# s-elkazdadi/ddp-pinocchio

Measured on AMD Instinct MI355X. Metric: DDP iterations/sec (fwd+bwd sweep), Talos nq=38 T=200, higher is better.
Workload: dtype f64

## Files before the change

ddp_pinocchio_amd/csrc/ctx.hip:

```cpp
#include <math.h>
#include <stdio.h>
#include <stdlib.h>
#include <string.h>

#include <limits>
#include <new>

#include "internal.h"

extern "C" int ddp_hip_abi_version(void) { return DDP_HIP_ABI_VERSION; }

extern "C" const char* ddp_hip_strerror(int code) {
  switch (code) {
    case DDP_HIP_OK: return "ok";
    case DDP_HIP_EV_LLT_RESTART: return "backward sweep restarted after a non-positive LLT pivot";
    case DDP_HIP_EV_LINESEARCH_FLOOR: return "line search reached step < 1e-10";
    case DDP_HIP_E_ARG: return "invalid argument";
    case DDP_HIP_E_HIP: return "HIP runtime error";
    case DDP_HIP_E_NODEVICE: return "no HIP device (there is no CPU fallback)";
    case DDP_HIP_E_UNSUPPORTED: return "unsupported configuration";
    case DDP_HIP_E_MAX_RESTARTS: return "backward sweep exceeded max_restarts";
    case DDP_HIP_E_COMM: return "RCCL error";
    default: return "unknown";
  }
// ... 157 lines not shown
         s == DDP_HIP_SEQ_FB_VAL || s == DDP_HIP_SEQ_FB_JAC || s == DDP_HIP_SEQ_X || s == DDP_HIP_SEQ_U ||
         s == DDP_HIP_SEQ_X_NEW || s == DDP_HIP_SEQ_U_NEW || is_trace_seq(s);
}

__global__ void fill_kernel(double* p, int64_t n, double v) {
  int64_t i = (int64_t)blockIdx.x * blockDim.x + threadIdx.x;
  int64_t stride = (int64_t)gridDim.x * blockDim.x;
  for (; i < n; i += stride) p[i] = v;
}

static int fill_device(ddp_hip_ctx* ctx, double* p, int64_t n, double v) {
  if (n <= 0) return DDP_HIP_OK;
  if (v == 0.0) {
    HIP_TRY(hipMemsetAsync(p, 0, (size_t)n * sizeof(double), ctx->stream));
    return DDP_HIP_OK;
  }
  int64_t blocks = (n + 255) / 256;
  if (blocks > 2048) blocks = 2048;
  hipLaunchKernelGGL(fill_kernel, dim3((unsigned)blocks), dim3(256), 0, ctx->stream, p, n, v);
  HIP_TRY(hipGetLastError());
  return DDP_HIP_OK;
}

static DevSwitches read_switches() {
  auto on = [](const char* name) { return getenv(name) != nullptr; };
  auto knob = [](const char* name, int lo, int hi) { const char* ev = getenv(name); const int v = ev ? atoi(ev) : 0; return v >= lo && v <= hi ? v : 0; };
  DevSwitches sw;
  sw.generic_bwd = on("DDP_HIP_GENERIC_BWD");
  sw.k3_no_sym = on("DDP_HIP_K3_NO_SYM");
  sw.k3_no_half = on("DDP_HIP_K3_NO_HALF");
  sw.k3_no_pack = on("DDP_HIP_K3_NO_PACK");
  sw.fxx_full = on("DDP_HIP_FXX_FULL");
  sw.no_static = on("DDP_HIP_NO_STATIC");
  sw.no_qcache = on("DDP_HIP_NO_QCACHE");
  sw.cfg_full_aba = on("DDP_HIP_CFG_FULL_ABA");
  sw.ana_own_aba = on("DDP_HIP_ANA_OWN_ABA");
  sw.ana_split = on("DDP_HIP_ANA_SPLIT");
  sw.ana_eq_kernel = on("DDP_HIP_ANA_EQ_KERNEL");
  sw.bwd_no_graph = on("DDP_HIP_BWD_NO_GRAPH");
  sw.solve_sync = on("DDP_HIP_SOLVE_SYNC");
  sw.fwd_no_pipe = on("DDP_HIP_FWD_NO_PIPE");
  sw.bwd_cbx = knob("DDP_HIP_BWD_CBX", 1, 8);
  sw.bwd_cbu = knob("DDP_HIP_BWD_CBU", 1, 16);
  sw.qws_bt = knob("DDP_HIP_QWS_BT", 16, 65536);
  sw.ana_bt = knob("DDP_HIP_ANA_BT", 1, 65536);
  return sw;
}

static int cost_block_setup(ddp_hip_ctx* ctx, int term, int32_t items) {
  CostBlock& k = ctx->cost[term];
  const int64_t slots = ctx->d.batch * (ctx->d.T + 1) * k.max_items;
  for (int s = 0; s < k.desc->nside; ++s) {
    const int64_t words = slots * k.desc->unit[s];
    const int fill = k.desc->fill[s];
    if (!k.side[s]) HIP_TRY(hipMalloc(&k.side[s], sizeof(double) * (size_t)words));
    if (fill == FILL_QUAT) {
      std::vector<double> qt((size_t)words, 0.0);
      for (size_t i = 3; i < qt.size(); i += 4) qt[i] = 1.0;
      HIP_TRY(hipMemcpyAsync(k.side[s], qt.data(), sizeof(double) * qt.size(), hipMemcpyHostToDevice, ctx->stream));
      HIP_TRY(hipStreamSynchronize(ctx->stream));
    } else {
      const int rc = fill_device(ctx, k.side[s], words, fill == FILL_NEG_INF ? -INFINITY : fill == FILL_POS_INF ? INFINITY : 0.0);
      if (rc != DDP_HIP_OK) return rc;
    }
  }
  k.items = items;
  k.live = false;
  return DDP_HIP_OK;
}

extern "C" int ddp_hip_create(const ddp_hip_problem* prob, int device, uint32_t flags, ddp_hip_ctx** out) {
// ... 566 lines not shown
```

ddp_pinocchio_amd/csrc/internal.h:

```cpp
#pragma once

#include <hip/hip_runtime.h>
#include <stdint.h>

#include <vector>

#include "cost_block.h"
#include "ddp_hip/ddp_hip.h"

#define DDP_MAXJ DDP_HIP_MAX_JOINTS

struct DevModel {
  int32_t kind, nv;
  int32_t ff, nj, nq, pad0_;
  double mass, length;
  double gravity[3];
  double dt, c;
  int32_t parent[DDP_MAXJ];
  int32_t jtype[DDP_MAXJ];
  double axis[DDP_MAXJ][3];
  double Rp[DDP_MAXJ][9];
  double pp[DDP_MAXJ][3];
  double I6[DDP_MAXJ][21];
  int32_t has_child[DDP_MAXJ];
// ... 23 lines not shown
};

struct BwdJob {
  int32_t kind;
  int32_t c0, cn;
  int32_t pad_;
};

struct DevSwitches {
  bool generic_bwd = false;
  bool k3_no_sym = false;
  bool k3_no_half = false;
  bool k3_no_pack = false;
  bool fxx_full = false;
  bool no_static = false;
  bool no_qcache = false;
  bool cfg_full_aba = false;
  bool ana_own_aba = false;
  bool ana_split = false;
  bool ana_eq_kernel = false;
  bool bwd_no_graph = false;
  bool solve_sync = false;
  bool fwd_no_pipe = false;
  int32_t bwd_cbx = 0, bwd_cbu = 0;
  int64_t qws_bt = 0;
  int64_t ana_bt = 0;
};

struct SweepPlan {
  bool fast;
  bool sym_ok;
  bool sym;
  int32_t half_mode;
  bool packed;
};

enum class LinFirst : int32_t {
  Base,
  AnalyticSmall,
  AnalyticWave,
  AnalyticFF,
  FdStatic,
  FdGeneric,
};
enum class LinSecond : int32_t {
  None,
  Zeros,
  Mode2Static,
  Mode2Caches,
  Mode2Plain,
  Mode1Small,
  Mode1Wave,
};
enum class LinEq : int32_t {
  None,
  PerLane,
  Analytic,
  Chain,
};
enum class LinEqJac : int32_t { None, Fd, FfLookahead };
enum class LinEqSecond : int32_t { None, Zeros, Mode2, Mode1Small, Mode1Wave };
struct LinPlan {
  int32_t refuse = 0;
  int32_t nj = 0;
  int32_t topo = 0;
  LinFirst first = LinFirst::Base;
  LinSecond second = LinSecond::None;
  LinEq eq = LinEq::None;
  LinEqJac eq_jac = LinEqJac::None;
  LinEqSecond eq_second = LinEqSecond::None;
  bool eq_inline = false;
  bool accel_static = false;
  bool accel_with_u = false;
  bool m1_fused = false;
  int32_t ncfg = 0, nvcfg = 0;
  bool has_tensors = false;
  bool skip_top = false;
  bool skip_qv_mirror = false;
  bool pack = false;
  bool ws_lin = false, ws_qws = false, ws_qws2 = false;
  bool ws_ana_T = false, ws_ana_M = false, ws_ana_M0 = false, ws_ana_A = false, ws_ana_F = false;
  bool ws_eq = false;
  bool ana_sliced = false;
  int64_t eq_fxk_off = 0, eq_c_off = 0, eq_words = 0;
  int32_t lin_path = 0, first_order = 0;
};
LinPlan lin_plan_decide(const DevModel& m, const Dims& d, uint32_t flags, const DevSwitches& sw, int topo_id, bool sweep_sym_ok);

enum class TensorOrigin : int32_t {
  Unknown,
  Symmetric,
  Stencil,
  Analytic1,
};
struct TensorState {
  TensorOrigin origin = TensorOrigin::Unknown;
  bool mirror_pending = false;
  bool packed = false;
};

struct LinCall {
  bool ana_A_fresh = false;
  bool ana_M0_fresh = false;
  bool fuu_zero = false;
};

struct ProfSlot {
  std::vector<hipEvent_t> starts, stops;
  size_t used = 0;
// ... 32 lines not shown
  struct BwdGraph { const void* key_x = nullptr; uint64_t key_misc = 0; hipGraphExec_t exec = nullptr; hipGraph_t graph = nullptr; };
  BwdGraph bwd_graph[4];
  int bwd_graph_next = 0;

  double* fw_x = nullptr;
  double* fw_u = nullptr;
  double* fw_dcost = nullptr;
  double* fw_cost = nullptr;
  double* fw_cost_old = nullptr;
  double* step_d = nullptr;
  int32_t* fw_state_d = nullptr;
  double* fw_dcost_acc_d = nullptr;
  int32_t n_alpha_max = 8;
  double* pick_pair_d = nullptr;

  double* eq_ws = nullptr;
  double* lin_ws = nullptr;
  LinPlan plan;
  double* lin_qws = nullptr;
  int64_t lin_qws_bt = 0;
  double* lin_qws2 = nullptr;
  hipStream_t lin_stream2 = nullptr;
  hipEvent_t lin_ev_up[2] = {nullptr, nullptr}, lin_ev_dn[2] = {nullptr, nullptr};
  double* ana_T = nullptr;
  double* ana_M = nullptr;
  double* ana_F = nullptr;
  double* ana_M0 = nullptr;
  double* ana_A = nullptr;
  int64_t ana_nbt = 0;

  std::vector<int32_t> active_h;
  bool all_active = true;

  CostBlock cost[COST_COUNT];
  int32_t fc_nf = 0;
  int32_t fc_joint[DDP_HIP_MAX_COST_FRAMES] = {};
  double fc_off[DDP_HIP_MAX_COST_FRAMES][3] = {};
  int32_t ob_np = 0, ob_no = 0;
  int32_t ob_joint[DDP_HIP_MAX_COLLISION_POINTS] = {};
  double ob_off[DDP_HIP_MAX_COLLISION_POINTS][3] = {};
  double ob_radius[DDP_HIP_MAX_COLLISION_POINTS] = {};
  int32_t ob_kind[DDP_HIP_MAX_OBSTACLES] = {};
  double* ob_clear_d = nullptr;

  bool box_dirty = false;

  bool async_mode = false;
  uint32_t profile_mask = 0;
  ProfSlot prof[DDP_HIP_K_COUNT];
};

#define HIP_TRY(expr)                                   \
  do {                                                  \
    hipError_t e__ = (expr);                            \
    if (e__ != hipSuccess) { (void)hipGetLastError(); return DDP_HIP_E_HIP; } \
  } while (0)

#define END_SYNC(ctx) do { if (!(ctx)->async_mode) HIP_TRY(hipStreamSynchronize((ctx)->stream)); } while (0)

void prof_begin(ddp_hip_ctx* ctx, int kid, hipStream_t stream = nullptr);
void prof_end(ddp_hip_ctx* ctx, int kid, hipStream_t stream = nullptr);

int bwd_setup(ddp_hip_ctx* ctx);
SweepPlan sweep_plan(const ddp_hip_ctx* ctx);
void bwd_teardown(ddp_hip_ctx* ctx);
int bwd_lds_check(const ddp_hip_ctx* ctx);
int box_check(ddp_hip_ctx* ctx);
int fwd_setup(ddp_hip_ctx* ctx);
bool fwd_lat_supported(const ddp_hip_ctx* ctx);
void fwd_teardown(ddp_hip_ctx* ctx);
int lin_setup(ddp_hip_ctx* ctx);
int tensors_written_outside(ddp_hip_ctx* ctx, int seq);
int lin_materialize_fxx(ddp_hip_ctx* ctx);
void lin_teardown(ddp_hip_ctx* ctx);

int pick_local_launch(ddp_hip_ctx* ctx, int64_t rank, int64_t nranks, double* out_pair, hipStream_t stream);
int pick_final_launch(const double* pairs, int G, double* out_pair, hipStream_t stream);

static inline int64_t seq_block_offset_regular(int64_t t, int64_t stride) { return t * stride; }
```

ddp_pinocchio_amd/csrc/lin.hip:

```cpp
#include <float.h>
#include <math.h>
#include <stdlib.h>

#include "com_cost.h"
#include "frame_cost.h"
#include "frame_vel_cost.h"
#include "internal.h"
#include "lin_common.h"
#include "obstacle_cost.h"
#include "rbd.h"
#include "rbd_deriv.h"
#include "state_limits.h"

namespace {



__global__ void lin_cost_kernel(LinParams p) {
  const int64_t T = p.d.T;
  const int64_t bt = blockIdx.x;
  const int b = (int)(bt / T);
  const int64_t t = bt % T;
  const int n = (int)p.d.n, m = (int)p.d.m;
  const double c = p.model->c;
// ... 1138 lines not shown
        const int rc_ = lin_analytic_launch(ctx, p, call, 0, LIN_ANA_F | (m1_next ? LIN_ANA_ACCEL : 0) | (m1_next && eq_stage ? LIN_ANA_EQ << 4 : 0));
        if (rc_ != DDP_HIP_OK) return rc_;
        break;
      }
      case LinFirst::FdStatic: {
        build_caches();
        const int rc_ = lin_static_launch(ctx, p, StaticLevel::FirstOrder);
        if (rc_ != DDP_HIP_OK) return rc_;
        break;
      }
      case LinFirst::FdGeneric:
        hipLaunchKernelGGL((lin_first_kernel<NJ>), dim3(blocks_for(BT * W)), dim3(LBS), 0, ctx->stream, p);
        break;
    }
    prof_end(ctx, DDP_HIP_K_LIN_FIRST);
  }
  if (second_stage) {
    const int64_t P = (int64_t)W * (W - 1) / 2, TRI = (int64_t)nv * (nv - 1) / 2, Pv = (int64_t)nv * nv + TRI, Pu = 2 * (int64_t)nv * nv + TRI;
    prof_begin(ctx, DDP_HIP_K_LIN_SECOND);
    switch (pl.second) {
      case LinSecond::None: break;
      case LinSecond::Mode2Static:
        build_caches();
        for (StaticLevel level : {StaticLevel::UDiagonal, StaticLevel::Torque, StaticLevel::Velocity, StaticLevel::Configuration}) {
          const int rc_ = lin_static_launch(ctx, p, level);
          if (rc_ != DDP_HIP_OK) return rc_;
        }
        break;
      case LinSecond::Mode2Caches:
        build_caches();
        hipLaunchKernelGGL((lin_diag_kernel<NJ>), dim3(blocks_for(BT * W)), dim3(LBS), 0, ctx->stream, p);
        hipLaunchKernelGGL((lin_offdiag_kernel<NJ, 3>), dim3(blocks_for(BT * Pu)), dim3(LBS), 0, ctx->stream, p);
        hipLaunchKernelGGL((lin_offdiag_kernel<NJ, 2>), dim3(blocks_for(BT * Pv)), dim3(LBS), 0, ctx->stream, p);
        hipLaunchKernelGGL((lin_offdiag_kernel<NJ, 1>), dim3(blocks_for(BT * TRI)), dim3(LBS), 0, ctx->stream, p);
        break;
      case LinSecond::Mode2Plain:
        hipLaunchKernelGGL((lin_diag_kernel<NJ>), dim3(blocks_for(BT * W)), dim3(LBS), 0, ctx->stream, p);
        hipLaunchKernelGGL((lin_offdiag_kernel<NJ, 0>), dim3(blocks_for(BT * P)), dim3(LBS), 0, ctx->stream, p);
        break;
      case LinSecond::Mode1Small:
        if constexpr (small) hipLaunchKernelGGL((second_m1_kernel<NJ>), dim3(blocks_for(BT * W)), dim3(LBS), 0, ctx->stream, p, 0);
        break;
      case LinSecond::Mode1Wave:
        if (!m1_fused) { const int rc_ = lin_analytic_launch(ctx, p, call, 1, LIN_ANA_F); if (rc_ != DDP_HIP_OK) return rc_; }
        break;
      case LinSecond::Zeros:
        HIP_TRY(hipMemsetAsync(p.fxx, 0, sizeof(double) * (size_t)(ctx->seq[DDP_HIP_SEQ_FXX].size * d.batch), ctx->stream));
        HIP_TRY(hipMemsetAsync(p.fux, 0, sizeof(double) * (size_t)(ctx->seq[DDP_HIP_SEQ_FUX].size * d.batch), ctx->stream));
        HIP_TRY(hipMemsetAsync(p.fuu, 0, sizeof(double) * (size_t)(ctx->seq[DDP_HIP_SEQ_FUU].size * d.batch), ctx->stream));
        break;
    }
    prof_end(ctx, DDP_HIP_K_LIN_SECOND);
  }
  if (eq_stage) {
    switch (pl.eq) {
      case LinEq::None: break;
      case LinEq::PerLane:
        if constexpr (small) hipLaunchKernelGGL((eq_first_kernel<NJ>), dim3(blocks_for(BT)), dim3(LBS), 0, ctx->stream, p);
        break;
      case LinEq::Analytic: {
        const int rc_ = lin_analytic_launch(ctx, p, call, 0, LIN_ANA_EQ);
        if (rc_ != DDP_HIP_OK) return rc_;
        break;
      }
      case LinEq::Chain: {
        const int K = ctx->model_h.eq_advance;
        if (K < 1) return DDP_HIP_E_UNSUPPORTED;
        hipLaunchKernelGGL((eq_chain_kernel<NJ>), dim3(blocks_for(BT)), dim3(LBS), 0, ctx->stream, p);
        if (pl.eq_jac == LinEqJac::Fd) hipLaunchKernelGGL((eq_fdjac_kernel<NJ>), dim3(blocks_for(BT * (K - 1) * d.n)), dim3(LBS), 0, ctx->stream, p);
        else if (pl.eq_jac == LinEqJac::FfLookahead) { const int rc_ = lin_analytic_ff_lookahead(ctx, p); if (rc_ != DDP_HIP_OK) return rc_; }
        hipLaunchKernelGGL(eq_combine_kernel, dim3((unsigned)BT), dim3(256), sizeof(double) * (size_t)(2 * d.emax * d.n), ctx->stream, p);
        break;
      }
    }
// ... 20 lines not shown
  return DDP_HIP_OK;
}

void tensors_end_second(ddp_hip_ctx* ctx, const LinParams& p, const LinCall& call) {
  TensorState& t = ctx->tensors;
  if (ctx->model_h.fd_mode == 1) t.origin = call.fuu_zero ? TensorOrigin::Analytic1 : TensorOrigin::Unknown;
  else t.origin = p.skip_top ? TensorOrigin::Stencil : TensorOrigin::Symmetric;
  t.mirror_pending = p.skip_qv_mirror != 0;
  t.packed = p.pack != 0;
}

}

int lin_setup(ddp_hip_ctx* ctx) {
  const Dims& d = ctx->d;
  const int topo_id = ctx->model_h.kind == DDP_HIP_MODEL_TREE ? lin_static_supported(ctx->model_h) : 0;
  ctx->plan = lin_plan_decide(ctx->model_h, d, ctx->flags, ctx->sw, topo_id, sweep_plan(ctx).sym_ok);
  const LinPlan& pl = ctx->plan;
  if (pl.refuse) return pl.refuse;
  if (pl.ws_lin)
    HIP_TRY(hipMalloc(&ctx->lin_ws, sizeof(double) * (size_t)(d.batch * d.T * ((int64_t)pl.ncfg * d.nv * rbd::QC_STRIDE + (int64_t)pl.nvcfg * d.nv * rbd::VC_STRIDE))));
  if (pl.ws_qws) {
    const int64_t BT = d.batch * d.T;
    int64_t slice = 1024;
    if (ctx->sw.qws_bt) slice = ctx->sw.qws_bt;
    ctx->lin_qws_bt = BT < slice ? BT : slice;
    HIP_TRY(hipMalloc(&ctx->lin_qws, sizeof(double) * (size_t)(ctx->lin_qws_bt * lin_static_ws_per_bt(ctx->model_h))));
    if (pl.ws_qws2) {
      HIP_TRY(hipMalloc(&ctx->lin_qws2, sizeof(double) * (size_t)(ctx->lin_qws_bt * lin_static_ws_per_bt(ctx->model_h))));
      HIP_TRY(hipStreamCreateWithFlags(&ctx->lin_stream2, hipStreamNonBlocking));
      for (int k = 0; k < 2; ++k) {
        HIP_TRY(hipEventCreateWithFlags(&ctx->lin_ev_up[k], hipEventDisableTiming));
        HIP_TRY(hipEventCreateWithFlags(&ctx->lin_ev_dn[k], hipEventDisableTiming));
      }
    }
  }
  { const int rc_ = lin_analytic_setup(ctx); if (rc_ != DDP_HIP_OK) return rc_; }
  if (pl.ws_eq) HIP_TRY(hipMalloc(&ctx->eq_ws, sizeof(double) * (size_t)pl.eq_words));
  if (pl.eq == LinEq::Chain) {
    const size_t lds = sizeof(double) * (size_t)(2 * d.emax * d.n);
    if (lds > 64 * 1024) HIP_TRY(hipFuncSetAttribute(reinterpret_cast<const void*>(&eq_combine_kernel), hipFuncAttributeMaxDynamicSharedMemorySize, (int)lds));
  }
  return DDP_HIP_OK;
}
void lin_teardown(ddp_hip_ctx* ctx) {
  lin_analytic_teardown(ctx);
  for (int k = 0; k < 2; ++k) {
    if (ctx->lin_ev_up[k]) (void)hipEventDestroy(ctx->lin_ev_up[k]);
    if (ctx->lin_ev_dn[k]) (void)hipEventDestroy(ctx->lin_ev_dn[k]);
  }
  if (ctx->lin_stream2) (void)hipStreamDestroy(ctx->lin_stream2);
  if (ctx->lin_qws2) (void)hipFree(ctx->lin_qws2);
  if (ctx->lin_qws) (void)hipFree(ctx->lin_qws);
  if (ctx->eq_ws) (void)hipFree(ctx->eq_ws);
  if (ctx->lin_ws) (void)hipFree(ctx->lin_ws);
}

extern "C" int ddp_hip_linearize_stages(ddp_hip_ctx* ctx, uint32_t stages) {
  if (!ctx) return DDP_HIP_E_ARG;
  HIP_TRY(hipSetDevice(ctx->device));
  LinParams p = make_params(ctx);
  LinCall call;
  const bool second = (stages & DDP_HIP_LIN_SECOND) && p.has_tensors;
  if (second) { const int rc_ = tensors_begin_second(ctx, p, call); if (rc_ != DDP_HIP_OK) return rc_; }
  int rc;
  switch (ctx->plan.nj) {
    case 1: rc = run_linearize<1>(ctx, p, call, stages); break;
    case 6: rc = run_linearize<6>(ctx, p, call, stages); break;
    case 38: rc = run_linearize<38>(ctx, p, call, stages); break;
    default: rc = run_linearize<64>(ctx, p, call, stages); break;
  }
  if (rc != DDP_HIP_OK) return rc;
  END_SYNC(ctx);
  if (second) tensors_end_second(ctx, p, call);
  return DDP_HIP_OK;
}

int tensors_written_outside(ddp_hip_ctx* ctx, int seq) {
  if (seq != DDP_HIP_SEQ_FXX && seq != DDP_HIP_SEQ_FUX && seq != DDP_HIP_SEQ_FUU) return DDP_HIP_OK;
  TensorState& t = ctx->tensors;
  if (t.packed) { const int rc_ = lin_materialize_fxx(ctx); if (rc_ != DDP_HIP_OK) return rc_; }
  if (seq == DDP_HIP_SEQ_FUX) {
    t.origin = (t.origin == TensorOrigin::Symmetric || t.origin == TensorOrigin::Stencil) ? TensorOrigin::Symmetric : TensorOrigin::Unknown;
    return DDP_HIP_OK;
  }
// ... 35 lines not shown
```

ddp_pinocchio_amd/csrc/lin_common.h:

```cpp
#pragma once
#include "internal.h"

struct LinParams {
  Dims d;
  const DevModel* model;
  const int64_t* ne;
  const int64_t* Epre;
  const double* target;
  const double *x, *u;
  double *lfx, *lfxx, *lx, *lu, *lxx, *lux, *luu;
  double *f_val, *fx, *fu, *fxx, *fux, *fuu;
  double *eq_val, *eq_x, *eq_u, *eq_xx, *eq_ux, *eq_uu;
  int32_t has_tensors;
  double *eq_xk, *eq_fxk, *eq_c;
  double* vcache;
  double* qcache;
  int32_t skip_qv_mirror;
  int32_t skip_top;
  int32_t pack;
  double* accel_out;
  int32_t ncfg, nvcfg;
  const double *xref, *wx, *uref, *wu;
};

constexpr int LBS = 64;

int lin_static_supported(const DevModel& m);
enum class StaticLevel {
  Caches,
  FirstOrder,
  UDiagonal,
  Torque,
  Velocity,
  Configuration,
  AccelX,
  AccelXU,
};
int lin_static_launch(ddp_hip_ctx* ctx, const LinParams& p, StaticLevel level);
int64_t lin_static_ws_per_bt(const DevModel& m);

int lin_analytic_setup(ddp_hip_ctx* ctx);
void lin_analytic_teardown(ddp_hip_ctx* ctx);
constexpr int LIN_ANA_F = 1, LIN_ANA_EQ = 2;
constexpr int LIN_ANA_ACCEL = 4;
int lin_analytic_launch(ddp_hip_ctx* ctx, const LinParams& p, LinCall& call, int stage, int flags);
int lin_analytic_ff_lookahead(ddp_hip_ctx* ctx, const LinParams& p);
```

ddp_pinocchio_amd/csrc/lin_plan.cpp:

```cpp
#include "internal.h"

LinPlan lin_plan_decide(const DevModel& m, const Dims& d, uint32_t flags, const DevSwitches& sw, int topo_id, bool sweep_sym_ok) {
  LinPlan pl;
  const bool tree = m.kind == DDP_HIP_MODEL_TREE, ff = m.ff != 0, fo_fd = m.first_order_fd != 0;
  const bool tensors = !(flags & DDP_HIP_FLAG_NO_TENSORS);
  const bool analytic = tree && !fo_fd;
  const int mode = m.fd_mode;
  const int64_t nv = d.nv, K = m.eq_advance;
  pl.has_tensors = tensors;
  pl.nj = nv <= 1 ? 1 : (nv <= 6 && !ff) ? 6 : nv <= 38 ? 38 : 64;
  const bool small = pl.nj <= 6;
  const bool wave = analytic && !small && !ff;

  if (mode == 1 && fo_fd && tensors) pl.refuse = DDP_HIP_E_UNSUPPORTED;
  if (analytic && ff && nv > 38) pl.refuse = DDP_HIP_E_UNSUPPORTED;
  if (wave && m.max_level_width > 64) pl.refuse = DDP_HIP_E_UNSUPPORTED;
  if (wave && d.Etot > 0 && (K < 1 || K > 2)) pl.refuse = DDP_HIP_E_UNSUPPORTED;

  const int topo = (tree && !ff && !sw.no_static) ? topo_id : 0;
  const bool stencil_caches = tree && mode == 2 && tensors && !ff && !sw.no_qcache;
  const bool accel = topo && wave && mode == 1 && tensors && !sw.ana_own_aba;
  if (stencil_caches) { pl.ncfg = (int32_t)nv + 1; pl.nvcfg = 2 * (int32_t)nv + 1; }
  else if ((topo && fo_fd) || accel) { pl.ncfg = 1; pl.nvcfg = 1; }
  pl.ws_lin = pl.ncfg > 0;
// ... 17 lines not shown
  const bool m1_wave = wave && pl.second == LinSecond::Mode1Wave;
  pl.ana_sliced = analytic && !small;
  pl.ws_ana_T = wave && sw.ana_split;
  pl.ws_ana_M = wave && (sw.ana_split || (m1_wave && d.Etot > 0));
  pl.ws_ana_M0 = m1_wave && !sw.ana_split;
  pl.ws_ana_A = pl.accel_static = accel;
  pl.accel_with_u = accel && d.Etot > 0;
  pl.ws_ana_F = m1_wave && d.Etot > 0;

  pl.ws_eq = d.Etot > 0 && tree && (fo_fd || ff);
  if (d.Etot > 0) {
    pl.eq = (small && !pl.ws_eq) ? LinEq::PerLane : wave ? LinEq::Analytic : LinEq::Chain;
    if (pl.eq == LinEq::Chain && K > 1) pl.eq_jac = fo_fd ? LinEqJac::Fd : LinEqJac::FfLookahead;
    pl.eq_second = !tensors ? LinEqSecond::None : mode == 0 ? LinEqSecond::Zeros : mode == 2 ? LinEqSecond::Mode2
                   : small ? LinEqSecond::Mode1Small : LinEqSecond::Mode1Wave;
    pl.m1_fused = m1_wave;
    pl.eq_inline = m1_wave && !sw.ana_split && m.eq_kind == DDP_HIP_EQ_CONFIG && !sw.ana_eq_kernel;
  }
  if (pl.ws_eq) {
    pl.eq_fxk_off = d.batch * d.T * K * d.nx;
    pl.eq_c_off = pl.eq_fxk_off + d.batch * d.T * (K > 1 ? K - 1 : 0) * d.n * d.n;
    pl.eq_words = pl.eq_c_off + d.batch * d.T * d.emax * d.n;
  }
  pl.lin_path = tree ? 1 + pl.topo : 0;
  pl.first_order = tree ? (fo_fd ? 1 : 2) : 0;
  return pl;
}

#ifdef LIN_PLAN_TABLE
#include <stdio.h>

int main() {
  static const char* const sw_names[] = {"none", "generic_bwd", "k3_no_sym", "k3_no_half", "fxx_full", "no_static", "no_qcache",
                                         "cfg_full_aba", "ana_own_aba", "ana_split", "ana_eq_kernel", "bwd_no_graph", "solve_sync"};
  printf("kind nv ff fo_fd mode tensors etot eq_kind K matched sw sym_ok created refuse nj topo first second eq eq_jac eq_second "
         "eq_inline accel_static accel_with_u m1_fused ncfg nvcfg has_tensors skip_top skip_qv_mirror pack ws_lin ws_qws ws_qws2 ws_ana_T "
         "ws_ana_M ws_ana_M0 ws_ana_A ws_ana_F ws_eq ana_sliced eq_fxk_off eq_c_off eq_words lin_path first_order\n");
  printf("#");
  for (const char* s : sw_names) printf(" %s", s);
  printf("\n");
  const int nvs[] = {1, 6, 7, 38, 39, 64};
  for (int kind : {DDP_HIP_MODEL_PENDULUM, DDP_HIP_MODEL_TREE})
  for (int nv : nvs) for (int ff = 0; ff < 2; ++ff) for (int fo = 0; fo < 2; ++fo) for (int mode = 0; mode < 3; ++mode)
  for (int tensors = 0; tensors < 2; ++tensors) for (int etot = 0; etot < 2; ++etot)
  for (int eqk : {DDP_HIP_EQ_NONE, DDP_HIP_EQ_CONFIG, DDP_HIP_EQ_FRAME}) for (int K = 1; K <= 3; ++K)
  for (int matched = 0; matched < 2; ++matched) for (int s = 0; s < 13; ++s) {
    DevModel m{};
    m.kind = kind; m.nv = nv; m.ff = ff; m.nj = ff ? nv - 5 : nv; m.nq = nv + ff;
    m.first_order_fd = fo; m.fd_mode = mode; m.eq_kind = eqk; m.eq_advance = K; m.max_level_width = 4;
    Dims d{};
    d.T = 3; d.batch = 2; d.nv = nv; d.n = 2 * nv; d.m = nv; d.nx = 2 * nv + ff;
    d.emax = etot ? (eqk == DDP_HIP_EQ_CONFIG ? nv : 3) : 0; d.Etot = etot ? d.emax * d.T : 0;
    DevSwitches sw;
    bool* const sws[] = {nullptr, &sw.generic_bwd, &sw.k3_no_sym, &sw.k3_no_half, &sw.fxx_full, &sw.no_static, &sw.no_qcache,
                         &sw.cfg_full_aba, &sw.ana_own_aba, &sw.ana_split, &sw.ana_eq_kernel, &sw.bwd_no_graph, &sw.solve_sync};
// ... 16 lines not shown
```

ddp_pinocchio_amd/csrc/lin_static.hip:

```cpp
#include <float.h>
#include <math.h>
#include <stdlib.h>

#include <type_traits>
#include <utility>

#include "internal.h"
#include "lin_common.h"
#include "rbd.h"

#ifndef DEV_NO_EMIT
#define DEV_NO_EMIT 0
#endif
namespace {

struct TopoTalos38 {
  static constexpr int N = 38;
  static constexpr int parent[N] = {-1, 0, 1, 2, 3, 4,
                                    5, 6, 7, 8, 9, 10,
                                    5, 12, 13, 14, 15, 16,
                                    5, 18,
                                    19, 20, 21, 22, 23, 24, 25, 26,
                                    19, 28, 29, 30, 31, 32, 33, 34,
                                    19, 36};
// ... 667 lines not shown
  }
#pragma unroll
  for (int k = 0; k < 6; ++k) vel[k] += vJ[k];
  rbd::crm(vel, vJ, cb);
  double sum = 0;
#pragma unroll
  for (int k = 0; k < 6; ++k) { ap[k] += cb[k]; sum += U[k] * ap[k]; }
  double ui;
  if constexpr (C::UQS == 0) ui = s.uu[K]; else ui = c.uq[K * C::UQS];
  const double qd = (ui - sum) * dinv;
  if constexpr (C::UQS == 0) s.uu[K] = qd; else c.uq[K * C::UQS] = qd;
  if constexpr (has_child<T>(K)) {
#pragma unroll
    for (int k = 0; k < 6; ++k) { s.vel[K][k] = vel[k]; s.acc[K][k] = ap[k]; }
    s.acc[K][o] += a[0] * qd; s.acc[K][o + 1] += a[1] * qd; s.acc[K][o + 2] += a[2] * qd;
  }
  __builtin_amdgcn_sched_barrier(0);
}
template <class T, class C, int... Ks>
__device__ __forceinline__ void vel_down_all(const C& c, VelState<T>& s, std::integer_sequence<int, Ks...>) {
  (vel_down<T, Ks>(c, s), ...);
}

template <class T, bool ROWS>
__global__ __launch_bounds__(LBS, ROWS ? 3 : 2) void lin_static_vel_kernel(LinParams p) {
  constexpr int nv = T::N, n = 2 * nv;
  constexpr int TRI = nv * (nv - 1) / 2, GU = (TRI + LBS - 1) / LBS, G = ROWS ? nv : GU;
  const int64_t bt = blockIdx.x / G;
  const int g = (int)(blockIdx.x % G);
  const int lane = threadIdx.x;
  const int64_t Tn = p.d.T;
  const int b = (int)(bt / Tn);
  const int64_t t = bt % Tn;
  int i, j, cfg;
  bool valid;
  if (ROWS) { i = g; j = nv + lane; cfg = 1 + g; valid = lane < nv; }
  else {
    const int pid = g * LBS + lane;
    valid = pid < TRI;
    tri_index(valid ? pid : 0, nv, i, j);
    i += nv; j += nv; cfg = 0;
  }
  struct PairStage { OutStage<nv, LBS / 2> O; double spare[nv + 1]; };
  using Stage = typename std::conditional<ROWS, RowStage<nv>, PairStage>::type;
  __shared__ union VelLds { Stage S; double P[nv * rbd::QC_STRIDE]; } s_lds;
  Stage& S = s_lds.S;
  double* s_P = s_lds.P;
  VelCtx<0, rbd::QC_STRIDE> c;
// ... 936 lines not shown
      const auto anc = [&](int a, int x) { for (int k = m.parent[x]; k >= 0; k = m.parent[k]) if (k == a) return true; return false; };
      int a = m.parent[i];
      while (a >= 0 && !anc(a, j)) a = m.parent[a];
      for (; a >= 0; a = m.parent[a]) ++rec;
    }
  const int64_t sweep = GU * nv * WS_PER_JOINT * LBS, splice = rec * SREC;
  return sweep > splice ? sweep : splice;
}

template <class T>
static void launch_first_columns(ddp_hip_ctx* ctx, const LinParams& p, bool with_u) {
  const int64_t BT = ctx->d.batch * ctx->d.T;
  constexpr int nv = T::N, TRI = nv * (nv - 1) / 2, GU = (TRI + LBS - 1) / LBS;
  const int64_t per = ctx->lin_qws_bt * GU;
  for (int64_t bt0 = 0; bt0 < BT; bt0 += per) {
    const int64_t nb = BT - bt0 < per ? BT - bt0 : per;
    hipLaunchKernelGGL((lin_static_first_kernel<T, 1, false>), dim3((unsigned)nb), dim3(LBS), 0, ctx->stream, p, p.model, p.qcache, p.x, p.u, ctx->lin_qws, bt0);
  }
  hipLaunchKernelGGL((lin_static_first_kernel<T, 2, false>), dim3((unsigned)BT), dim3(LBS), 0, ctx->stream, p, p.model, p.qcache, p.x, p.u, ctx->lin_qws, (int64_t)0);
  if (with_u) hipLaunchKernelGGL((lin_static_first_kernel<T, 3, false>), dim3((unsigned)BT), dim3(LBS), 0, ctx->stream, p, p.model, p.qcache, p.x, p.u, ctx->lin_qws, (int64_t)0);
}

template <class T>
static int lin_static_launch_t(ddp_hip_ctx* ctx, const LinParams& p, StaticLevel level) {
  const int64_t BT = ctx->d.batch * ctx->d.T;
  constexpr int nv = T::N, TRI = nv * (nv - 1) / 2, GU = (TRI + LBS - 1) / LBS;
  if (level == StaticLevel::Torque) {
    hipLaunchKernelGGL((lin_static_tau_kernel<T, true>), dim3((unsigned)(BT * 2 * nv)), dim3(LBS), 0, ctx->stream, p);
    if (p.pack) hipLaunchKernelGGL((lin_static_tau_kernel<T, false, true>), dim3((unsigned)(BT * GU)), dim3(LBS), 0, ctx->stream, p);
    else hipLaunchKernelGGL((lin_static_tau_kernel<T, false, false>), dim3((unsigned)(BT * GU)), dim3(LBS), 0, ctx->stream, p);
  } else if (level == StaticLevel::Caches) {
    hipLaunchKernelGGL((lin_static_qvcache_kernel<T>), dim3((unsigned)((BT * p.ncfg + LBS - 1) / LBS)), dim3(LBS), 0, ctx->stream, p, p.model, p.x, p.qcache, p.vcache);
    if (p.nvcfg > 1) hipLaunchKernelGGL((lin_static_vcache_kernel<T>), dim3((unsigned)BT), dim3(LBS), 0, ctx->stream, p, p.model, p.x, p.qcache, p.vcache);
  } else if (level == StaticLevel::AccelXU || level == StaticLevel::AccelX) {
    if (!p.accel_out) return DDP_HIP_E_ARG;
    hipLaunchKernelGGL((lin_static_qvcache_kernel<T>), dim3((unsigned)((BT * p.ncfg + LBS - 1) / LBS)), dim3(LBS), 0, ctx->stream, p, p.model, p.x, p.qcache, p.vcache);
    launch_first_columns<T>(ctx, p, level == StaticLevel::AccelXU);
  } else if (level == StaticLevel::FirstOrder) {
    launch_first_columns<T>(ctx, p, true);
  } else if (level == StaticLevel::UDiagonal) {
    hipLaunchKernelGGL((lin_static_first_kernel<T, 3, true>), dim3((unsigned)BT), dim3(LBS), 0, ctx->stream, p, p.model, p.qcache, p.x, p.u, ctx->lin_qws, (int64_t)0);
  } else if (level == StaticLevel::Configuration && !ctx->sw.cfg_full_aba) {
    constexpr int64_t NREC = spine_records<T>(), SWEEP = (int64_t)GU * nv * WS_PER_JOINT * LBS;
    constexpr int64_t WS_BT = SWEEP > NREC * SREC ? SWEEP : NREC * SREC;
    const int64_t per = NREC > 0 ? ctx->lin_qws_bt * WS_BT / (NREC * SREC) : BT;
    for (int64_t bt0 = 0; bt0 < BT; bt0 += per) {
      const int nb = (int)(BT - bt0 < per ? BT - bt0 : per);
      const dim3 grid((unsigned)((nb + 7) / 8 * 8 * GU));
      hipLaunchKernelGGL((lin_static_spine_kernel<T>), grid, dim3(LBS), 0, ctx->stream, p.model, p.qcache, p.vcache, ctx->lin_qws, bt0, nb);
      hipLaunchKernelGGL((lin_static_cfg_pair_kernel<T>), grid, dim3(LBS), 0, ctx->stream, p, ctx->lin_qws, bt0, nb);
    }
  } else if (level == StaticLevel::Configuration) {
    const int64_t per = ctx->lin_qws_bt;
    hipStream_t s0 = ctx->stream, s1 = ctx->lin_stream2;
    int k = 0;
    for (int64_t bt0 = 0; bt0 < BT; bt0 += per, ++k) {
      const int64_t nb = BT - bt0 < per ? BT - bt0 : per;
      const int w = k & 1;
      double* ws = w ? ctx->lin_qws2 : ctx->lin_qws;
      if (k >= 2) HIP_TRY(hipStreamWaitEvent(s0, ctx->lin_ev_dn[w], 0));
      hipLaunchKernelGGL((lin_static_cfg_up_kernel<T>), dim3((unsigned)(nb * GU)), dim3(LBS), 0, s0, p, p.model, p.qcache, p.x, p.u, ws, bt0);
      HIP_TRY(hipEventRecord(ctx->lin_ev_up[w], s0));
      HIP_TRY(hipStreamWaitEvent(s1, ctx->lin_ev_up[w], 0));
      hipLaunchKernelGGL((lin_static_cfg_down_kernel<T>), dim3((unsigned)(nb * GU)), dim3(LBS), 0, s1, p, p.model, p.qcache, p.x, p.u, ws, bt0);
      HIP_TRY(hipEventRecord(ctx->lin_ev_dn[w], s1));
    }
    if (k >= 1) HIP_TRY(hipStreamWaitEvent(s0, ctx->lin_ev_dn[0], 0));
    if (k >= 2) HIP_TRY(hipStreamWaitEvent(s0, ctx->lin_ev_dn[1], 0));
  } else if (level == StaticLevel::Velocity) {
    hipLaunchKernelGGL((lin_static_vel_kernel<T, true>), dim3((unsigned)(BT * nv)), dim3(LBS), 0, ctx->stream, p);
    hipLaunchKernelGGL((lin_static_vel_kernel<T, false>), dim3((unsigned)(BT * GU)), dim3(LBS), 0, ctx->stream, p);
  }
  HIP_TRY(hipGetLastError());
  return DDP_HIP_OK;
// ... 11 lines not shown
```

Baseline: 745.5.

## Fork configuration-level static second-order kernels onto a side stream

Adds a SecondOrder static level that launches the u-diagonal, torque, velocity and configuration kernels together. The spine and configuration-pair kernels go to a second stream, forked and joined with events, so they overlap with the torque and velocity kernels on the main stream. When the spine fork is on, the qws slice size grows from 1024 to 3200 so fewer, larger slices run. This trades more workspace memory and extra stream and event management for concurrency. The spine kernel may also start early and race on shared workspace if the event ordering is wrong.

```diff
diff --git a/ddp_pinocchio_amd/csrc/ctx.hip b/ddp_pinocchio_amd/csrc/ctx.hip
--- a/ddp_pinocchio_amd/csrc/ctx.hip
+++ b/ddp_pinocchio_amd/csrc/ctx.hip
@@ -203,31 +203,6 @@
   return DDP_HIP_OK;
 }
 
-static DevSwitches read_switches() {
-  auto on = [](const char* name) { return getenv(name) != nullptr; };
-  auto knob = [](const char* name, int lo, int hi) { const char* ev = getenv(name); const int v = ev ? atoi(ev) : 0; return v >= lo && v <= hi ? v : 0; };
-  DevSwitches sw;
-  sw.generic_bwd = on("DDP_HIP_GENERIC_BWD");
-  sw.k3_no_sym = on("DDP_HIP_K3_NO_SYM");
-  sw.k3_no_half = on("DDP_HIP_K3_NO_HALF");
-  sw.k3_no_pack = on("DDP_HIP_K3_NO_PACK");
-  sw.fxx_full = on("DDP_HIP_FXX_FULL");
-  sw.no_static = on("DDP_HIP_NO_STATIC");
-  sw.no_qcache = on("DDP_HIP_NO_QCACHE");
-  sw.cfg_full_aba = on("DDP_HIP_CFG_FULL_ABA");
-  sw.ana_own_aba = on("DDP_HIP_ANA_OWN_ABA");
-  sw.ana_split = on("DDP_HIP_ANA_SPLIT");
-  sw.ana_eq_kernel = on("DDP_HIP_ANA_EQ_KERNEL");
-  sw.bwd_no_graph = on("DDP_HIP_BWD_NO_GRAPH");
-  sw.solve_sync = on("DDP_HIP_SOLVE_SYNC");
-  sw.fwd_no_pipe = on("DDP_HIP_FWD_NO_PIPE");
-  sw.bwd_cbx = knob("DDP_HIP_BWD_CBX", 1, 8);
-  sw.bwd_cbu = knob("DDP_HIP_BWD_CBU", 1, 16);
-  sw.qws_bt = knob("DDP_HIP_QWS_BT", 16, 65536);
-  sw.ana_bt = knob("DDP_HIP_ANA_BT", 1, 65536);
-  return sw;
-}
-
 static int cost_block_setup(ddp_hip_ctx* ctx, int term, int32_t items) {
   CostBlock& k = ctx->cost[term];
   const int64_t slots = ctx->d.batch * (ctx->d.T + 1) * k.max_items;
diff --git a/ddp_pinocchio_amd/csrc/internal.h b/ddp_pinocchio_amd/csrc/internal.h
--- a/ddp_pinocchio_amd/csrc/internal.h
+++ b/ddp_pinocchio_amd/csrc/internal.h
@@ -69,6 +69,8 @@
   bool bwd_no_graph = false;
   bool solve_sync = false;
   bool fwd_no_pipe = false;
+  bool lin_serial = false;
+  int32_t lin_forks = 0;
   int32_t bwd_cbx = 0, bwd_cbu = 0;
   int64_t qws_bt = 0;
   int64_t ana_bt = 0;
@@ -104,6 +106,11 @@
   PerLane,
   Analytic,
   Chain,
+};
+enum LinFork : uint32_t {
+  LIN_FORK_CFG = 1,
+  LIN_FORK_SPINE = 2,
+  LIN_FORK_DEFAULT = LIN_FORK_CFG | LIN_FORK_SPINE,
 };
 enum class LinEqJac : int32_t { None, Fd, FfLookahead };
 enum class LinEqSecond : int32_t { None, Zeros, Mode2, Mode1Small, Mode1Wave };
@@ -130,8 +137,10 @@
   bool ws_eq = false;
   bool ana_sliced = false;
   int64_t eq_fxk_off = 0, eq_c_off = 0, eq_words = 0;
+  uint32_t forks = 0;
   int32_t lin_path = 0, first_order = 0;
 };
+DevSwitches read_switches();
 LinPlan lin_plan_decide(const DevModel& m, const Dims& d, uint32_t flags, const DevSwitches& sw, int topo_id, bool sweep_sym_ok);
 
 enum class TensorOrigin : int32_t {
@@ -210,6 +219,8 @@
   double* lin_qws2 = nullptr;
   hipStream_t lin_stream2 = nullptr;
   hipEvent_t lin_ev_up[2] = {nullptr, nullptr}, lin_ev_dn[2] = {nullptr, nullptr};
+  hipEvent_t lin_ev_fork = nullptr, lin_ev_done = nullptr, lin_ev_rows = nullptr;
+  bool lin_side_busy = false;
   double* ana_T = nullptr;
   double* ana_M = nullptr;
   double* ana_F = nullptr;
@@ -245,6 +256,28 @@
   } while (0)
 
 #define END_SYNC(ctx) do { if (!(ctx)->async_mode) HIP_TRY(hipStreamSynchronize((ctx)->stream)); } while (0)
+
+inline hipError_t lin_fork(ddp_hip_ctx* ctx) {
+  hipError_t e = hipEventRecord(ctx->lin_ev_fork, ctx->stream);
+  if (e == hipSuccess) e = hipStreamWaitEvent(ctx->lin_stream2, ctx->lin_ev_fork, 0);
+  if (e == hipSuccess) ctx->lin_side_busy = true;
+  return e;
+}
+inline hipError_t lin_join(ddp_hip_ctx* ctx) {
+  if (!ctx->lin_side_busy) return hipSuccess;
+  hipError_t e = hipEventRecord(ctx->lin_ev_done, ctx->lin_stream2);
+  if (e == hipSuccess) e = hipStreamWaitEvent(ctx->stream, ctx->lin_ev_done, 0);
+  if (e != hipSuccess) { (void)hipGetLastError(); (void)hipStreamSynchronize(ctx->lin_stream2); }
+  ctx->lin_side_busy = false;
+  return e;
+}
+struct LinJoin {
+  ddp_hip_ctx* ctx;
+  explicit LinJoin(ddp_hip_ctx* c) : ctx(c) {}
+  LinJoin(const LinJoin&) = delete;
+  LinJoin& operator=(const LinJoin&) = delete;
+  ~LinJoin() { (void)lin_join(ctx); }
+};
 
 void prof_begin(ddp_hip_ctx* ctx, int kid, hipStream_t stream = nullptr);
 void prof_end(ddp_hip_ctx* ctx, int kid, hipStream_t stream = nullptr);
diff --git a/ddp_pinocchio_amd/csrc/lin.hip b/ddp_pinocchio_amd/csrc/lin.hip
--- a/ddp_pinocchio_amd/csrc/lin.hip
+++ b/ddp_pinocchio_amd/csrc/lin.hip
@@ -1184,6 +1184,11 @@
       case LinSecond::None: break;
       case LinSecond::Mode2Static:
         build_caches();
+        if (pl.forks) {
+          const int rc_ = lin_static_launch(ctx, p, StaticLevel::SecondOrder);
+          if (rc_ != DDP_HIP_OK) return rc_;
+          break;
+        }
         for (StaticLevel level : {StaticLevel::UDiagonal, StaticLevel::Torque, StaticLevel::Velocity, StaticLevel::Configuration}) {
           const int rc_ = lin_static_launch(ctx, p, level);
           if (rc_ != DDP_HIP_OK) return rc_;
@@ -1212,6 +1217,7 @@
         HIP_TRY(hipMemsetAsync(p.fuu, 0, sizeof(double) * (size_t)(ctx->seq[DDP_HIP_SEQ_FUU].size * d.batch), ctx->stream));
         break;
     }
+    HIP_TRY(lin_join(ctx));
     prof_end(ctx, DDP_HIP_K_LIN_SECOND);
   }
   if (eq_stage) {
@@ -1278,7 +1284,7 @@
     HIP_TRY(hipMalloc(&ctx->lin_ws, sizeof(double) * (size_t)(d.batch * d.T * ((int64_t)pl.ncfg * d.nv * rbd::QC_STRIDE + (int64_t)pl.nvcfg * d.nv * rbd::VC_STRIDE))));
   if (pl.ws_qws) {
     const int64_t BT = d.batch * d.T;
-    int64_t slice = 1024;
+    int64_t slice = (pl.forks & LIN_FORK_SPINE) ? 3200 : 1024;
     if (ctx->sw.qws_bt) slice = ctx->sw.qws_bt;
     ctx->lin_qws_bt = BT < slice ? BT : slice;
     HIP_TRY(hipMalloc(&ctx->lin_qws, sizeof(double) * (size_t)(ctx->lin_qws_bt * lin_static_ws_per_bt(ctx->model_h))));
@@ -1291,6 +1297,12 @@
       }
     }
   }
+  if (pl.forks) {
+    HIP_TRY(hipStreamCreateWithFlags(&ctx->lin_stream2, hipStreamNonBlocking));
+    HIP_TRY(hipEventCreateWithFlags(&ctx->lin_ev_fork, hipEventDisableTiming));
+    HIP_TRY(hipEventCreateWithFlags(&ctx->lin_ev_done, hipEventDisableTiming));
+    HIP_TRY(hipEventCreateWithFlags(&ctx->lin_ev_rows, hipEventDisableTiming));
+  }
   { const int rc_ = lin_analytic_setup(ctx); if (rc_ != DDP_HIP_OK) return rc_; }
   if (pl.ws_eq) HIP_TRY(hipMalloc(&ctx->eq_ws, sizeof(double) * (size_t)pl.eq_words));
   if (pl.eq == LinEq::Chain) {
@@ -1305,6 +1317,7 @@
     if (ctx->lin_ev_up[k]) (void)hipEventDestroy(ctx->lin_ev_up[k]);
     if (ctx->lin_ev_dn[k]) (void)hipEventDestroy(ctx->lin_ev_dn[k]);
   }
+  for (hipEvent_t ev : {ctx->lin_ev_fork, ctx->lin_ev_done, ctx->lin_ev_rows}) if (ev) (void)hipEventDestroy(ev);
   if (ctx->lin_stream2) (void)hipStreamDestroy(ctx->lin_stream2);
   if (ctx->lin_qws2) (void)hipFree(ctx->lin_qws2);
   if (ctx->lin_qws) (void)hipFree(ctx->lin_qws);
@@ -1317,6 +1330,7 @@
   HIP_TRY(hipSetDevice(ctx->device));
   LinParams p = make_params(ctx);
   LinCall call;
+  LinJoin joined(ctx);
   const bool second = (stages & DDP_HIP_LIN_SECOND) && p.has_tensors;
   if (second) { const int rc_ = tensors_begin_second(ctx, p, call); if (rc_ != DDP_HIP_OK) return rc_; }
   int rc;
diff --git a/ddp_pinocchio_amd/csrc/lin_common.h b/ddp_pinocchio_amd/csrc/lin_common.h
--- a/ddp_pinocchio_amd/csrc/lin_common.h
+++ b/ddp_pinocchio_amd/csrc/lin_common.h
@@ -33,6 +33,7 @@
   Torque,
   Velocity,
   Configuration,
+  SecondOrder,
   AccelX,
   AccelXU,
 };
diff --git a/ddp_pinocchio_amd/csrc/lin_plan.cpp b/ddp_pinocchio_amd/csrc/lin_plan.cpp
--- a/ddp_pinocchio_amd/csrc/lin_plan.cpp
+++ b/ddp_pinocchio_amd/csrc/lin_plan.cpp
@@ -1,4 +1,33 @@
+#include <stdlib.h>
+
 #include "internal.h"
+
+DevSwitches read_switches() {
+  auto on = [](const char* name) { return getenv(name) != nullptr; };
+  auto knob = [](const char* name, int lo, int hi) { const char* ev = getenv(name); const int v = ev ? atoi(ev) : 0; return v >= lo && v <= hi ? v : 0; };
+  DevSwitches sw;
+  sw.generic_bwd = on("DDP_HIP_GENERIC_BWD");
+  sw.k3_no_sym = on("DDP_HIP_K3_NO_SYM");
+  sw.k3_no_half = on("DDP_HIP_K3_NO_HALF");
+  sw.k3_no_pack = on("DDP_HIP_K3_NO_PACK");
+  sw.fxx_full = on("DDP_HIP_FXX_FULL");
+  sw.no_static = on("DDP_HIP_NO_STATIC");
+  sw.no_qcache = on("DDP_HIP_NO_QCACHE");
+  sw.cfg_full_aba = on("DDP_HIP_CFG_FULL_ABA");
+  sw.ana_own_aba = on("DDP_HIP_ANA_OWN_ABA");
+  sw.ana_split = on("DDP_HIP_ANA_SPLIT");
+  sw.ana_eq_kernel = on("DDP_HIP_ANA_EQ_KERNEL");
+  sw.bwd_no_graph = on("DDP_HIP_BWD_NO_GRAPH");
+  sw.solve_sync = on("DDP_HIP_SOLVE_SYNC");
+  sw.fwd_no_pipe = on("DDP_HIP_FWD_NO_PIPE");
+  sw.lin_serial = on("DDP_HIP_LIN_SERIAL");
+  sw.lin_forks = knob("DDP_HIP_LIN_FORKS", 1, 3);
+  sw.bwd_cbx = knob("DDP_HIP_BWD_CBX", 1, 8);
+  sw.bwd_cbu = knob("DDP_HIP_BWD_CBU", 1, 16);
+  sw.qws_bt = knob("DDP_HIP_QWS_BT", 16, 65536);
+  sw.ana_bt = knob("DDP_HIP_ANA_BT", 1, 65536);
+  return sw;
+}
 
 LinPlan lin_plan_decide(const DevModel& m, const Dims& d, uint32_t flags, const DevSwitches& sw, int topo_id, bool sweep_sym_ok) {
   LinPlan pl;
@@ -63,6 +92,7 @@
     pl.eq_c_off = pl.eq_fxk_off + d.batch * d.T * (K > 1 ? K - 1 : 0) * d.n * d.n;
     pl.eq_words = pl.eq_c_off + d.batch * d.T * d.emax * d.n;
   }
+  if (pl.second == LinSecond::Mode2Static && !sw.lin_serial && !sw.cfg_full_aba) pl.forks = sw.lin_forks ? (uint32_t)sw.lin_forks : (uint32_t)LIN_FORK_DEFAULT;
   pl.lin_path = tree ? 1 + pl.topo : 0;
   pl.first_order = tree ? (fo_fd ? 1 : 2) : 0;
   return pl;
@@ -71,7 +101,16 @@
 #ifdef LIN_PLAN_TABLE
 #include <stdio.h>
 
-int main() {
+int main(int argc, char** argv) {
+  if (argc > 1 && argv[1][0] == 's') {
+    DevModel m{};
+    m.kind = DDP_HIP_MODEL_TREE; m.nv = 38; m.nj = 38; m.nq = 38; m.first_order_fd = 1; m.fd_mode = 2; m.max_level_width = 4;
+    Dims d{};
+    d.T = 3; d.batch = 2; d.nv = 38; d.n = 76; d.m = 38; d.nx = 76;
+    const LinPlan p = lin_plan_decide(m, d, 0u, read_switches(), 1, true);
+    printf("forks %u topo %d\n", p.forks, p.topo);
+    return 0;
+  }
   static const char* const sw_names[] = {"none", "generic_bwd", "k3_no_sym", "k3_no_half", "fxx_full", "no_static", "no_qcache",
                                          "cfg_full_aba", "ana_own_aba", "ana_split", "ana_eq_kernel", "bwd_no_graph", "solve_sync"};
   printf("kind nv ff fo_fd mode tensors etot eq_kind K matched sw sym_ok created refuse nj topo first second eq eq_jac eq_second "
diff --git a/ddp_pinocchio_amd/csrc/lin_static.hip b/ddp_pinocchio_amd/csrc/lin_static.hip
--- a/ddp_pinocchio_amd/csrc/lin_static.hip
+++ b/ddp_pinocchio_amd/csrc/lin_static.hip
@@ -713,8 +713,11 @@
   (vel_down<T, Ks>(c, s), ...);
 }
 
+#ifndef DDP_VEL_PAIR_WAVES
+#define DDP_VEL_PAIR_WAVES 2
+#endif
 template <class T, bool ROWS>
-__global__ __launch_bounds__(LBS, ROWS ? 3 : 2) void lin_static_vel_kernel(LinParams p) {
+__global__ __launch_bounds__(LBS, ROWS ? 3 : DDP_VEL_PAIR_WAVES) void lin_static_vel_kernel(LinParams p) {
   constexpr int nv = T::N, n = 2 * nv;
   constexpr int TRI = nv * (nv - 1) / 2, GU = (TRI + LBS - 1) / LBS, G = ROWS ? nv : GU;
   const int64_t bt = blockIdx.x / G;
@@ -1697,6 +1700,46 @@
 }
 
 template <class T>
+static int launch_cfg_slices(ddp_hip_ctx* ctx, const LinParams& p, hipStream_t s, hipEvent_t rows_done) {
+  const int64_t BT = ctx->d.batch * ctx->d.T;
+  constexpr int nv = T::N, TRI = nv * (nv - 1) / 2, GU = (TRI + LBS - 1) / LBS;
+  constexpr int64_t NREC = spine_records<T>(), SWEEP = (int64_t)GU * nv * WS_PER_JOINT * LBS;
+  constexpr int64_t WS_BT = SWEEP > NREC * SREC ? SWEEP : NREC * SREC;
+  const int64_t per = NREC > 0 ? ctx->lin_qws_bt * WS_BT / (NREC * SREC) : BT;
+  for (int64_t bt0 = 0; bt0 < BT; bt0 += per) {
+    const int nb = (int)(BT - bt0 < per ? BT - bt0 : per);
+    const dim3 grid((unsigned)((nb + 7) / 8 * 8 * GU));
+    hipLaunchKernelGGL((lin_static_spine_kernel<T>), grid, dim3(LBS), 0, s, p.model, p.qcache, p.vcache, ctx->lin_qws, bt0, nb);
+    if (rows_done) { HIP_TRY(hipStreamWaitEvent(s, rows_done, 0)); rows_done = nullptr; }
+    hipLaunchKernelGGL((lin_static_cfg_pair_kernel<T>), grid, dim3(LBS), 0, s, p, ctx->lin_qws, bt0, nb);
+  }
+  return DDP_HIP_OK;
+}
+
+template <class T>
+static int launch_second_order(ddp_hip_ctx* ctx, const LinParams& p) {
+  const int64_t BT = ctx->d.batch * ctx->d.T;
+  constexpr int nv = T::N, TRI = nv * (nv - 1) / 2, GU = (TRI + LBS - 1) / LBS;
+  const bool fork_cfg = (ctx->plan.forks & LIN_FORK_CFG) != 0, spine_ahead = fork_cfg && (ctx->plan.forks & LIN_FORK_SPINE);
+  hipStream_t s0 = ctx->stream;
+  if (spine_ahead) HIP_TRY(lin_fork(ctx));
+  hipLaunchKernelGGL((lin_static_first_kernel<T, 3, true>), dim3((unsigned)BT), dim3(LBS), 0, s0, p, p.model, p.qcache, p.x, p.u, ctx->lin_qws, (int64_t)0);
+  hipLaunchKernelGGL((lin_static_tau_kernel<T, true>), dim3((unsigned)(BT * 2 * nv)), dim3(LBS), 0, s0, p);
+  if (fork_cfg) {
+    if (spine_ahead) HIP_TRY(hipEventRecord(ctx->lin_ev_rows, s0));
+    else HIP_TRY(lin_fork(ctx));
+    const int rc_ = launch_cfg_slices<T>(ctx, p, ctx->lin_stream2, spine_ahead ? ctx->lin_ev_rows : nullptr);
+    if (rc_ != DDP_HIP_OK) return rc_;
+  }
+  if (p.pack) hipLaunchKernelGGL((lin_static_tau_kernel<T, false, true>), dim3((unsigned)(BT * GU)), dim3(LBS), 0, s0, p);
+  else hipLaunchKernelGGL((lin_static_tau_kernel<T, false, false>), dim3((unsigned)(BT * GU)), dim3(LBS), 0, s0, p);
+  hipLaunchKernelGGL((lin_static_vel_kernel<T, true>), dim3((unsigned)(BT * nv)), dim3(LBS), 0, s0, p);
+  hipLaunchKernelGGL((lin_static_vel_kernel<T, false>), dim3((unsigned)(BT * GU)), dim3(LBS), 0, s0, p);
+  if (!fork_cfg) { const int rc_ = launch_cfg_slices<T>(ctx, p, s0, nullptr); if (rc_ != DDP_HIP_OK) return rc_; }
+  return DDP_HIP_OK;
+}
+
+template <class T>
 static int lin_static_launch_t(ddp_hip_ctx* ctx, const LinParams& p, StaticLevel level) {
   const int64_t BT = ctx->d.batch * ctx->d.T;
   constexpr int nv = T::N, TRI = nv * (nv - 1) / 2, GU = (TRI + LBS - 1) / LBS;
@@ -1713,18 +1756,12 @@
     launch_first_columns<T>(ctx, p, level == StaticLevel::AccelXU);
   } else if (level == StaticLevel::FirstOrder) {
     launch_first_columns<T>(ctx, p, true);
+  } else if (level == StaticLevel::SecondOrder) {
+    { const int rc_ = launch_second_order<T>(ctx, p); if (rc_ != DDP_HIP_OK) return rc_; }
   } else if (level == StaticLevel::UDiagonal) {
     hipLaunchKernelGGL((lin_static_first_kernel<T, 3, true>), dim3((unsigned)BT), dim3(LBS), 0, ctx->stream, p, p.model, p.qcache, p.x, p.u, ctx->lin_qws, (int64_t)0);
   } else if (level == StaticLevel::Configuration && !ctx->sw.cfg_full_aba) {
-    constexpr int64_t NREC = spine_records<T>(), SWEEP = (int64_t)GU * nv * WS_PER_JOINT * LBS;
-    constexpr int64_t WS_BT = SWEEP > NREC * SREC ? SWEEP : NREC * SREC;
-    const int64_t per = NREC > 0 ? ctx->lin_qws_bt * WS_BT / (NREC * SREC) : BT;
-    for (int64_t bt0 = 0; bt0 < BT; bt0 += per) {
-      const int nb = (int)(BT - bt0 < per ? BT - bt0 : per);
-      const dim3 grid((unsigned)((nb + 7) / 8 * 8 * GU));
-      hipLaunchKernelGGL((lin_static_spine_kernel<T>), grid, dim3(LBS), 0, ctx->stream, p.model, p.qcache, p.vcache, ctx->lin_qws, bt0, nb);
-      hipLaunchKernelGGL((lin_static_cfg_pair_kernel<T>), grid, dim3(LBS), 0, ctx->stream, p, ctx->lin_qws, bt0, nb);
-    }
+    { const int rc_ = launch_cfg_slices<T>(ctx, p, ctx->stream, nullptr); if (rc_ != DDP_HIP_OK) return rc_; }
   } else if (level == StaticLevel::Configuration) {
     const int64_t per = ctx->lin_qws_bt;
     hipStream_t s0 = ctx->stream, s1 = ctx->lin_stream2;
```

New measurement: 770.9 (median of 6 runs). +3.4%, better.
